# nagadomi/nunif

Hardware: NVIDIA H100
Metric: waifu2x_input_megapixels_per_sec (higher is better)
Workload: dtype f16

## Files before the change

nunif_b200/csrc/gemm_wgmma.cuh:

```cuda
#pragma once
#include "common.cuh"
#include <cuda.h>

namespace nb200 {

enum : int { ACT_NONE = 0, ACT_LRELU01 = 1, ACT_GELU = 2, ACT_RELU = 3 };
enum : int { OUT_NHWC = 0, OUT_PIXSHUF2 = 1, OUT_SPLIT = 2 };

struct GemmParams {
    int B, Ho, Wo, TH, TW, tiles_x, tiles_y;
    int N;
    int taps, cpt;
    int8_t tap_dx[16], tap_dy[16], tap_dyi[16];
    int n_tiles;
    const float* bias;
    int act;
    int out_mode, cout;
    int has_res, res_cy, res_cx;
    int res_before_act;
};

struct GemmMaps {
    CUtensorMap a, b;
    CUtensorMap o[4];
    CUtensorMap r[4];
};

__device__ __forceinline__ uint32_t smem_u32(const void* p) { return (uint32_t)__cvta_generic_to_shared(p); }

__device__ __forceinline__ void mbar_init(uint64_t* bar, uint32_t count) {
    asm volatile("mbarrier.init.shared::cta.b64 [%0], %1;" ::"r"(smem_u32(bar)), "r"(count));
}
__device__ __forceinline__ void mbar_expect_tx(uint64_t* bar, uint32_t bytes) {
    asm volatile("mbarrier.arrive.expect_tx.shared::cta.b64 _, [%0], %1;" ::"r"(smem_u32(bar)), "r"(bytes) : "memory");
}
__device__ __forceinline__ void mbar_arrive(uint64_t* bar) {
    asm volatile("mbarrier.arrive.shared::cta.b64 _, [%0];" ::"r"(smem_u32(bar)) : "memory");
}
static __device__ __noinline__ void mbar_timeout() {
    printf("nb200: mbarrier wait timed out (block %d,%d thread %d)\n", blockIdx.x, blockIdx.y, threadIdx.x);
    __trap();
}
__device__ __forceinline__ void mbar_wait(uint64_t* bar, uint32_t parity) {
    const uint32_t addr = smem_u32(bar);
    uint32_t done = 0;
#pragma unroll 1
    for (uint32_t it = 0; it < (1u << 18); ++it) {
        asm volatile(
            "{\n\t.reg .pred p;\n\t"
            "mbarrier.try_wait.parity.shared::cta.b64 p, [%1], %2, %3;\n\t"
            "selp.u32 %0, 1, 0, p;\n\t}"
            : "=r"(done) : "r"(addr), "r"(parity), "r"(20000u) : "memory");
        if (done) return;
    }
    mbar_timeout();
}
__device__ __forceinline__ void fence_barrier_init() {
    asm volatile("fence.mbarrier_init.release.cluster;" ::: "memory");
    asm volatile("fence.proxy.async.shared::cta;" ::: "memory");
}
__device__ __forceinline__ void tma_load_5d(const CUtensorMap* map, uint64_t* bar, void* dst, int c0, int c1, int c2, int c3, int c4) {
    asm volatile(
        "cp.async.bulk.tensor.5d.shared::cluster.global.tile.mbarrier::complete_tx::bytes [%0], [%1, {%3, %4, %5, %6, %7}], [%2];"
        ::"r"(smem_u32(dst)), "l"(map), "r"(smem_u32(bar)), "r"(c0), "r"(c1), "r"(c2), "r"(c3), "r"(c4) : "memory");
}
__device__ __forceinline__ void tma_load_2d(const CUtensorMap* map, uint64_t* bar, void* dst, int c0, int c1) {
    asm volatile(
        "cp.async.bulk.tensor.2d.shared::cluster.global.tile.mbarrier::complete_tx::bytes [%0], [%1, {%3, %4}], [%2];"
        ::"r"(smem_u32(dst)), "l"(map), "r"(smem_u32(bar)), "r"(c0), "r"(c1) : "memory");
}
__device__ __forceinline__ void tma_load_4d(const CUtensorMap* map, uint64_t* bar, void* dst, int c0, int c1, int c2, int c3) {
    asm volatile(
        "cp.async.bulk.tensor.4d.shared::cluster.global.tile.mbarrier::complete_tx::bytes [%0], [%1, {%3, %4, %5, %6}], [%2];"
        ::"r"(smem_u32(dst)), "l"(map), "r"(smem_u32(bar)), "r"(c0), "r"(c1), "r"(c2), "r"(c3) : "memory");
}
__device__ __forceinline__ void tma_store_4d(const CUtensorMap* map, const void* src, int c0, int c1, int c2, int c3) {
    asm volatile("cp.async.bulk.tensor.4d.global.shared::cta.tile.bulk_group [%0, {%2, %3, %4, %5}], [%1];"
                 ::"l"(map), "r"(smem_u32(src)), "r"(c0), "r"(c1), "r"(c2), "r"(c3) : "memory");
// ... 282 lines not shown
```

nunif_b200/csrc/model.cu:

```cuda
#include "common.cuh"
#include "gemm.h"
#include "gemm_wgmma.cuh"
#include "swin_kernels.h"
#include "cunet_kernels.h"
#include "legacy_kernels.h"
#include "depth_kernels.h"
#include "rowflow_kernels.h"
#include "depth_aa_kernels.h"
#include "mlbw_kernels.h"
#include "zoe_kernels.h"
#include "inpaint_kernels.h"
#include "window_mha.h"
#include "sod_kernels.h"
#include "../../include/nunif_b200.h"
#include <map>
#include <vector>
#include <string>
#include <cstring>
#include <cmath>
#include <memory>
#include <tuple>
#include <algorithm>

namespace nb200 {
// ... 260 lines not shown
        Arena size;
        plan(size);
        if (ensure_ws(size.off + 4096)) return 1;
        Arena a{ws};
        plan(a);
        return 0;
    }
};

namespace nb200 {

static void pack_swin_blocks(Packer& pk, std::vector<SwinBlockW>& out, const std::string& prefix, int C, int layers) {
    for (int i = 0; i < layers; ++i) {
        SwinBlockW b;
        const std::string p = prefix + ".block." + std::to_string(i);
        b.C = C;
        b.shift = (i % 2 == 0) ? 0 : 3;
        b.qkv = pack_linear(pk, p + ".attn.qkv", 3 * C, C);
        b.proj = pack_linear(pk, p + ".attn.proj", C, C);
        b.fc1 = pack_linear(pk, p + ".mlp.0", 2 * C, C);
        b.fc2 = pack_linear(pk, p + ".mlp.3", C, 2 * C);
        const float* t = pk.get(p + ".attn.relative_position_bias_table", 121 * 6);
        if (t) {
            std::vector<float> frag(BIAS_FRAG_FLOATS);
            for (int head = 0; head < 6; ++head)
                for (int mt = 0; mt < 3; ++mt)
                    for (int nt = 0; nt < 6; ++nt)
                        for (int lane = 0; lane < 32; ++lane)
                            for (int r = 0; r < 4; ++r) {
                                const int g = lane >> 2, t4 = lane & 3;
                                const int row = mt * 16 + g + 8 * (r >> 1), col = nt * 8 + 2 * t4 + (r & 1);
                                float v;
                                if (col >= 36) v = -1e30f;
                                else if (row >= 36) v = 0.f;
                                else {
                                    const int qy = row / 6, qx = row % 6, ky = col / 6, kx = col % 6;
                                    v = 1.4426950408889634f * t[((qy - ky + 5) * 11 + (qx - kx + 5)) * 6 + head];
                                }
                                frag[((((size_t)head * 3 + mt) * 6 + nt) * 32 + lane) * 4 + r] = v;
                            }
            b.table = pk.add_f32(frag);
        }
        pk.mark(p + ".attn.relative_position_index");
        out.push_back(b);
    }
}

static void pack_swin(Packer& pk, SwinW& w, int r) {
    const int C = 96;
    w.C = C;
    w.r = r;
    w.cs = (3 * r * r + 15) / 16 * 16;
    w.stem = pack_stem(pk, "unet.patch.0", C / 2, 64);
    w.conv2 = pack_conv(pk, "unet.patch.2", C, C / 2, 3, 3, 64);
    pack_swin_blocks(pk, w.s1, "unet.swin1", C, 2);
    w.down1 = pack_conv(pk, "unet.down1.conv", 2 * C, C, 2, 2);
    pack_swin_blocks(pk, w.s2, "unet.swin2", 2 * C, 2);
    w.down2 = pack_conv(pk, "unet.down2.conv", 2 * C, 2 * C, 2, 2);
    pack_swin_blocks(pk, w.s3, "unet.swin3", 2 * C, 6);
    w.up2 = pack_linear_pixshuf2(pk, "unet.up2.proj", 2 * C, 2 * C);
    pack_swin_blocks(pk, w.s4, "unet.swin4", 2 * C, 2);
    if (r == 4) {
        w.proj2 = pack_linear(pk, "unet.proj2", 2 * C, C);
        w.up1 = pack_linear_pixshuf2(pk, "unet.up1.proj", 2 * C, 2 * C);
// ... 473 lines not shown
```

nunif_b200/csrc/swin_attention_mma.cu:

```cuda
#include "common.cuh"
#include "gemm_wgmma.cuh"
#include "swin_kernels.h"
#include "tmap.h"
#include <map>
#include <mutex>

namespace nb200 {

extern int g_tune[16];

namespace {
constexpr int WS = 6, WTOK = 36, WPAD = 48, HEADS = 6;

__device__ __forceinline__ void mma16816(float (&c)[4], const uint32_t (&a)[4], uint32_t b0, uint32_t b1) {
    asm volatile(
        "mma.sync.aligned.m16n8k16.row.col.f32.f16.f16.f32 {%0,%1,%2,%3}, {%4,%5,%6,%7}, {%8,%9}, {%0,%1,%2,%3};"
        : "+f"(c[0]), "+f"(c[1]), "+f"(c[2]), "+f"(c[3])
        : "r"(a[0]), "r"(a[1]), "r"(a[2]), "r"(a[3]), "r"(b0), "r"(b1));
}
__device__ __forceinline__ void ldmatrix_x2_trans(uint32_t& r0, uint32_t& r1, const void* smem_row) {
    const uint32_t addr = (uint32_t)__cvta_generic_to_shared(smem_row);
    asm volatile("ldmatrix.sync.aligned.m8n8.x2.trans.shared.b16 {%0,%1}, [%2];" : "=r"(r0), "=r"(r1) : "r"(addr));
}
__device__ __forceinline__ uint32_t pack_half2(float a, float b) {
// ... 255 lines not shown
int window_attention(cudaStream_t st, const __half* qkv, const float* bias_frag_f, __half* out, int B, int H, int W, int C,
                     int shift, size_t plane) {
    const float4* bias_table = reinterpret_cast<const float4*>(bias_frag_f);
    NB_CHECK(H % WS == 0 && W % WS == 0, "feature map must be a multiple of the 6x6 window");
    NB_CHECK(C == 96 || C == 192, "window attention supports C=96 (d=16) and C=192 (d=32)");
    if (WS >= H) shift = 0;
    dim3 grid((H / WS) * (W / WS), B);
    ProfScope ps(st, PC_ATTN, (double)B * H * W * C * 4 * 2, (double)B * H * W * C * 3 * 2, (double)B * H * W * C * 2);
    if (C == 96) {
        const int want = g_tune[6] > 0 ? g_tune[6] : 72;
        if (set_attn_attrs((const void*)window_attention_mma_kernel<16>, attn_smem_bytes<16>(), want)) return 1;
        window_attention_mma_kernel<16><<<grid, 192, attn_smem_bytes<16>(), st>>>(qkv, bias_table, out, H, W, shift, plane);
    } else {
        const int want = g_tune[6] > 0 ? g_tune[6] : 86;
        if (set_attn_attrs((const void*)window_attention_mma_kernel<32>, attn_smem_bytes<32>(), want)) return 1;
        window_attention_mma_kernel<32><<<grid, 192, attn_smem_bytes<32>(), st>>>(qkv, bias_table, out, H, W, shift, plane);
    }
    NB_LAUNCHED();
    return 0;
}


constexpr int FA_ROWS = 128, FA_WIN = 3, FA_THREADS = GEMM_CONSUMER_THREADS + 32, FA_SLOT = 96 * 64, FA_STAGES = 4;
constexpr int FA_LD = 32 + 8;
constexpr int FA_CHUNK_BYTES = FA_WIN * 3 * WTOK * FA_LD * 2;

template <int C>
struct FaCfg {
    static constexpr int X_BYTES = FA_ROWS * C * 2;
    static constexpr int SMEM = X_BYTES + FA_STAGES * FA_SLOT + FA_CHUNK_BYTES + FA_WIN * (WTOK + WPAD) * 4 + 2 * FA_STAGES * 8 + 1024;
};

template <int C>
__global__ void __launch_bounds__(FA_THREADS, 2) swin_attn_fused_kernel(const __grid_constant__ CUtensorMap wmap,
                                                                        const __half* __restrict__ x, const float* __restrict__ bqkv,
                                                                        const float4* __restrict__ bias_frag, __half* __restrict__ out,
                                                                        int H, int W, int shift, int nwin) {
    using Cfg = FaCfg<C>;
    constexpr int D = C / HEADS, KB = C / 32, NCH = C / 32, HPC = 32 / D;
    extern __shared__ uint8_t smem_dyn[];
    uint8_t* smem = reinterpret_cast<uint8_t*>((reinterpret_cast<uintptr_t>(smem_dyn) + 1023) & ~(uintptr_t)1023);
    uint8_t* sx = smem;
    uint8_t* ring = smem + Cfg::X_BYTES;
    __half* sqkv = reinterpret_cast<__half*>(ring + FA_STAGES * FA_SLOT);
    int* stok = reinterpret_cast<int*>(reinterpret_cast<uint8_t*>(sqkv) + FA_CHUNK_BYTES);
    int* sreg = stok + FA_WIN * WTOK;
    uint64_t* full = reinterpret_cast<uint64_t*>(sreg + FA_WIN * WPAD);
    uint64_t* empty = full + FA_STAGES;
    const int tid = threadIdx.x, warp = tid >> 5;
    const int nww = W / WS, nwy = H / WS;
    if (tid < FA_WIN * WPAD) {
        const int w = tid / WPAD, t = tid % WPAD, gw = blockIdx.x * FA_WIN + w;
        int reg = -1;
        if (t < WTOK) {
            int tok = -1;
            if (gw < nwin) {
                const int b = gw / (nww * nwy), r = gw % (nww * nwy), wy = r / nww, wx = r % nww;
                const int ry = wy * WS + t / WS, rx = wx * WS + t % WS;
                const int y = (ry + shift) % H, xx = (rx + shift) % W;
                tok = (b * H + y) * W + xx;
                int hr = 0, wr = 0;
                if (shift > 0) {
                    hr = ry < H - WS ? 0 : (ry < H - shift ? 1 : 2);
                    wr = rx < W - WS ? 0 : (rx < W - shift ? 1 : 2);
                }
                reg = hr * 3 + wr;
            }
            stok[w * WTOK + t] = tok;
// ... 12 lines not shown
    if (tid == 0) NB_PDL_TRIGGER();

    if (warp == GEMM_CONSUMER_THREADS / 32) {
        if (elect_one()) {
            for (int i = 0; i < NCH * KB; ++i) {
                const int s = i % FA_STAGES, c = i / KB;
                mbar_wait(&empty[s], ((i / FA_STAGES) & 1) ^ 1);
                mbar_expect_tx(&full[s], FA_SLOT);
#pragma unroll
                for (int m = 0; m < 3; ++m)
                    tma_load_2d(&wmap, &full[s], ring + s * FA_SLOT + m * 32 * 64, (i % KB) * 32, m * C + 32 * c);
            }
        }
        return;
    }

    for (int i = tid; i < FA_ROWS * (C / 8); i += GEMM_CONSUMER_THREADS) {
        const int r = i / (C / 8), u = i % (C / 8);
        uint8_t* dst = sx + (u >> 2) * (FA_ROWS * 64) + stage_off<32>(r, u & 3);
        const int tok = r < FA_WIN * WTOK ? stok[r] : -1;
        if (tok >= 0) cp_async16(dst, x + (size_t)tok * C + u * 8);
        else *reinterpret_cast<uint4*>(dst) = make_uint4(0u, 0u, 0u, 0u);
    }
    asm volatile("cp.async.commit_group;" ::: "memory");
    asm volatile("cp.async.wait_group 0;" ::: "memory");
    fence_async_smem();
    consumer_bar_sync();

    const int wg = tid >> 7, t = tid & 127;
    const int row0 = wg * 64 + (t >> 5) * 16 + ((t & 31) >> 2);
    const int cq = 2 * (t & 3);
    const uint32_t a_base = smem_u32(sx) + wg * 64 * 64;
    const int lane = tid & 31, g = lane >> 2, t4 = lane & 3;
    const float scale = ((D == 16) ? 0.25f : 0.17677669529663687f) * 1.4426950408889634f;
#pragma unroll 1
    for (int c = 0; c < NCH; ++c) {
        float acc[48];
#pragma unroll
        for (int j = 0; j < 48; ++j) acc[j] = 0.f;
#pragma unroll 1
        for (int kb = 0; kb < KB; ++kb) {
            const int it = c * KB + kb, s = it % FA_STAGES;
            mbar_wait(&full[s], (it / FA_STAGES) & 1);
            const uint32_t a = a_base + kb * (FA_ROWS * 64), bb = smem_u32(ring + s * FA_SLOT);
            wgmma_fence();
            wgmma_f16<96>(acc, make_kmajor_desc<64>(a), make_kmajor_desc<64>(bb), 1u);
            wgmma_f16<96>(acc, make_kmajor_desc<64>(a + 32), make_kmajor_desc<64>(bb + 32), 1u);
            wgmma_commit();
            wgmma_wait<1>();
            if (kb > 0 && t == 0) mbar_arrive(&empty[(it - 1) % FA_STAGES]);
        }
        wgmma_wait<0>();
        if (t == 0) mbar_arrive(&empty[(c * KB + KB - 1) % FA_STAGES]);
        wgmma_fence_operands(acc);
        consumer_bar_sync();
#pragma unroll
        for (int j = 0; j < 12; ++j) {
            const int m = j >> 2, col = 8 * (j & 3) + cq;
            const float2 bq = __ldg(reinterpret_cast<const float2*>(bqkv + m * C + 32 * c + col));
#pragma unroll
            for (int i = 0; i < 2; ++i) {
                const int r = row0 + 8 * i;
                if (r < FA_WIN * WTOK) {
                    const int w = r / WTOK, tk = r - w * WTOK;
                    *reinterpret_cast<__half2*>(sqkv + ((w * 3 + m) * WTOK + tk) * FA_LD + col) =
                        __floats2half2_rn(acc[4 * j + 2 * i] + bq.x, acc[4 * j + 2 * i + 1] + bq.y);
                }
            }
        }
        consumer_bar_sync();

#pragma unroll 1
        for (int item = warp; item < 3 * FA_WIN * HPC; item += GEMM_CONSUMER_THREADS / 32) {
            const int mt = item / (FA_WIN * HPC), pr = item - mt * (FA_WIN * HPC), w = pr / HPC, hh = pr - w * HPC;
            const int gw = blockIdx.x * FA_WIN + w;
            if (gw >= nwin) continue;
            const int r = gw % (nww * nwy), wy = r / nww, wx = r % nww, head = c * HPC + hh;
            __half* sq = sqkv + w * 3 * WTOK * FA_LD;
            __half* sk = sq + WTOK * FA_LD;
            __half* sv = sk + WTOK * FA_LD;
            AttnCtx<D> cx;
            cx.sq = sq; cx.sreg = sreg + w * WPAD; cx.bf = bias_frag + (size_t)head * (3 * 6 * 32) + lane;
            cx.hc = hh * D; cx.g = g; cx.t4 = t4; cx.scale = scale;
            cx.boundary = shift > 0 && (wy == nwy - 1 || wx == nww - 1);
#pragma unroll
            for (int nt = 0; nt < NKT; ++nt) cx.kbase[nt] = sk + min(nt * 8 + g, WTOK - 1) * FA_LD + cx.hc + 2 * t4;
            cx.vbase[0] = sv + (lane & 15) * FA_LD + cx.hc;
            cx.vbase[1] = sv + (16 + (lane & 15)) * FA_LD + cx.hc;
            cx.vbase[2] = sv + min(32 + (lane & 7), WTOK - 1) * FA_LD + cx.hc;
            if (mt < 2) attn_mtile<D, FA_LD, false>(cx, mt);
            else attn_mtile<D, FA_LD, true>(cx, 2);
            __syncwarp();
            const int nrow = mt < 2 ? 16 : WTOK - 32;
            for (int e = lane; e < nrow * (D / 8); e += 32) {
                const int tk = 16 * mt + e / (D / 8), u = e % (D / 8);
                *reinterpret_cast<uint4*>(out + (size_t)stok[w * WTOK + tk] * C + head * D + u * 8) =
                    *reinterpret_cast<const uint4*>(sq + tk * FA_LD + cx.hc + u * 8);
            }
        }
    }
}

int swin_attn_fused(cudaStream_t st, const __half* x, const __half* wqkv, const float* bqkv, const float* bias_frag_f, __half* att,
                    int B, int H, int W, int C, int shift) {
    NB_CHECK(x && wqkv && bqkv && bias_frag_f && att, "null pointer");
    NB_CHECK(H % WS == 0 && W % WS == 0, "feature map must be a multiple of the 6x6 window");
    NB_CHECK(C == 96 || C == 192, "fused window attention supports C=96 (d=16) and C=192 (d=32)");
    if (WS >= H) shift = 0;
    const long long nwin = (long long)B * (H / WS) * (W / WS);
    NB_CHECK(nwin > 0 && nwin < (1LL << 31), "window count out of range");
    CUtensorMap wmap;
    const cuuint64_t dims[2] = {(cuuint64_t)C, (cuuint64_t)(3 * C)};
    const cuuint64_t strides[1] = {(cuuint64_t)C * 2};
    const cuuint32_t box[2] = {32, 32};
    if (encode(&wmap, wqkv, 2, dims, strides, box, 64)) return 1;
    const double T = (double)B * H * W;
    ProfScope ps(st, PC_FUSED_ATTN, T * 3.0 * C * C * 2 + T * C * 36 * 4, T * C * 2, T * C * 2);
    const unsigned grid = (unsigned)((nwin + FA_WIN - 1) / FA_WIN);
    const float4* bf = reinterpret_cast<const float4*>(bias_frag_f);
    if (C == 96) {
        if (ensure_dyn_smem((const void*)swin_attn_fused_kernel<96>, FaCfg<96>::SMEM)) return 1;
        swin_attn_fused_kernel<96><<<grid, FA_THREADS, FaCfg<96>::SMEM, st>>>(wmap, x, bqkv, bf, att, H, W, shift, (int)nwin);
    } else {
        if (ensure_dyn_smem((const void*)swin_attn_fused_kernel<192>, FaCfg<192>::SMEM)) return 1;
        swin_attn_fused_kernel<192><<<grid, FA_THREADS, FaCfg<192>::SMEM, st>>>(wmap, x, bqkv, bf, att, H, W, shift, (int)nwin);
    }
    NB_LAUNCHED();
    return 0;
}

}
```

nunif_b200/csrc/swin_block.cu:

```cuda
#include "gemm_wgmma.cuh"
#include "swin_kernels.h"
#include "tmap.h"

namespace nb200 {

constexpr int FM_ROWS = 128, FM_STAGES = 5, FM_THREADS = GEMM_CONSUMER_THREADS + 128;
constexpr int FM_PRODUCER_REGS = 40, FM_CONSUMER_REGS = 232;

template <int C>
struct FmCfg {
    static constexpr int KB = C / 32;
    static constexpr int TILE = FM_ROWS * C * 2;
    static constexpr int STAGE = 128 * C;
    static constexpr int SMEM = 2 * TILE + FM_STAGES * STAGE + (2 * FM_STAGES + KB + 1) * 8 + 1024;
};

struct FmMaps {
    CUtensorMap x, att, wp, w1, w2;
};

template <int K>
__device__ __forceinline__ float (&half96(float (&acc)[K], int h))[48] { return *reinterpret_cast<float(*)[48]>(&acc[48 * h]); }

__device__ __forceinline__ void fm_wait(uint64_t* bar, uint32_t parity) {
    const uint32_t addr = smem_u32(bar);
    uint32_t done = 0;
#pragma unroll 1
    for (uint32_t it = 0; it < (1u << 18) && !done; ++it)
        asm volatile(
            "{\n\t.reg .pred p;\n\t"
            "mbarrier.try_wait.parity.shared::cta.b64 p, [%1], %2, %3;\n\t"
            "selp.u32 %0, 1, 0, p;\n\t}"
            : "=r"(done) : "r"(addr), "r"(parity), "r"(20000u) : "memory");
    if (!done) __trap();
}

__device__ __forceinline__ void wgmma_wait_n(int n) {
    if (n == 0) wgmma_wait<0>();
    else wgmma_wait<1>();
}

template <int C, bool PROJ>
__global__ void __launch_bounds__(FM_THREADS, 1) swin_mlp_fused_kernel(const __grid_constant__ FmMaps maps, const float* __restrict__ bp,
                                                                     const float* __restrict__ b1, const float* __restrict__ b2) {
    using Cfg = FmCfg<C>;
    constexpr int KB = Cfg::KB, NP = (KB + 1) / 2, NH = 2 * C / 64, NHALF = C / 96;
    extern __shared__ uint8_t smem_dyn[];
    uint8_t* smem = reinterpret_cast<uint8_t*>((reinterpret_cast<uintptr_t>(smem_dyn) + 1023) & ~(uintptr_t)1023);
    uint8_t* sx = smem;
    uint8_t* satt = smem + Cfg::TILE;
    uint8_t* ring = smem + 2 * Cfg::TILE;
    uint64_t* full = reinterpret_cast<uint64_t*>(ring + FM_STAGES * Cfg::STAGE);
    uint64_t* empty = full + FM_STAGES;
    uint64_t* abar = empty + FM_STAGES;
    uint64_t* xbar = abar + KB;
    const int tid = threadIdx.x, warp = tid >> 5;
    const int row_base = blockIdx.x * FM_ROWS;
    if (tid == GEMM_CONSUMER_THREADS) {
// ... 13 lines not shown
        fence_barrier_init();
    }
    __syncthreads();

    if (warp >= GEMM_CONSUMER_THREADS / 32) {
        asm volatile("setmaxnreg.dec.sync.aligned.u32 %0;" ::"n"(FM_PRODUCER_REGS));
        if (warp == GEMM_CONSUMER_THREADS / 32 && elect_one()) {
            bool acts = false;
            auto load_acts = [&]() {
                asm volatile("griddepcontrol.wait;" ::: "memory");
                if (PROJ)
                    for (int kb = 0; kb < KB; ++kb) {
                        mbar_expect_tx(&abar[kb], FM_ROWS * 64);
                        tma_load_2d(&maps.att, &abar[kb], satt + kb * (FM_ROWS * 64), kb * 32, row_base);
                    }
                mbar_expect_tx(xbar, Cfg::TILE);
                for (int kb = 0; kb < KB; ++kb) tma_load_2d(&maps.x, xbar, sx + kb * (FM_ROWS * 64), kb * 32, row_base);
                acts = true;
            };
            int it = 0;
            auto push = [&](const CUtensorMap* m, int k0, int n0, int rows, int nbox) {
                if (it == FM_STAGES) load_acts();
                const int s = it % FM_STAGES;
                fm_wait(&empty[s], ((it / FM_STAGES) & 1) ^ 1);
                mbar_expect_tx(&full[s], nbox * rows * 64);
                for (int b = 0; b < nbox; ++b) tma_load_2d(m, &full[s], ring + s * Cfg::STAGE + b * rows * 64, k0 + 32 * b, n0);
                ++it;
            };
            if (PROJ)
                for (int j = 0; j < NP; ++j) push(&maps.wp, 64 * j, 0, C, min(2, KB - 2 * j));
            push(&maps.w1, 0, 0, 64, KB);
            for (int hc = 0; hc < NH; ++hc) {
                if (hc + 1 < NH) push(&maps.w1, 0, (hc + 1) * 64, 64, KB);
                push(&maps.w2, hc * 64, 0, C, 2);
            }
            if (!acts) load_acts();
        }
        return;
    }

    asm volatile("setmaxnreg.inc.sync.aligned.u32 %0;" ::"n"(FM_CONSUMER_REGS));
    const int wg = tid >> 7, t = tid & 127;
    const int row0 = wg * 64 + (t >> 5) * 16 + ((t & 31) >> 2);
    const int cq = 2 * (t & 3);
    const uint32_t x_base = smem_u32(sx) + wg * 64 * 64, att_base = smem_u32(satt) + wg * 64 * 64;
    int it = 0, pending = 0;
    auto take = [&]() -> uint32_t {
        const int s = it % FM_STAGES;
        fm_wait(&full[s], (it / FM_STAGES) & 1);
        return smem_u32(ring + s * Cfg::STAGE);
    };
    auto commit = [&]() {
        wgmma_commit();
        ++it;
        ++pending;
    };
    auto retire = [&](int n) {
        wgmma_wait_n(n);
#pragma unroll
        for (int k = 0; k < FM_STAGES; ++k)
            if (k < pending - n && t == 0) mbar_arrive(&empty[(it - pending + k) % FM_STAGES]);
        pending = min(pending, n);
    };

    if (PROJ) {
        float acc[C / 2];
#pragma unroll
        for (int j = 0; j < C / 2; ++j) acc[j] = 0.f;
        wgmma_fence_operands(acc);
#pragma unroll
        for (int j = 0; j < NP; ++j) {
            const uint32_t bb = take();
#pragma unroll
            for (int kb = 2 * j; kb < 2 * j + 2 && kb < KB; ++kb) fm_wait(&abar[kb], 0);
            wgmma_fence();
#pragma unroll
            for (int kb = 2 * j; kb < 2 * j + 2 && kb < KB; ++kb) {
                const uint32_t a = att_base + kb * (FM_ROWS * 64), b = bb + (kb - 2 * j) * (C * 64);
#pragma unroll
                for (int s = 0; s < 2; ++s)
#pragma unroll
                    for (int h = 0; h < NHALF; ++h)
                        wgmma_f16<96>(half96(acc, h), make_kmajor_desc<64>(a + 32 * s), make_kmajor_desc<64>(b + h * 96 * 64 + 32 * s), 1u);
            }
            commit();
            retire(1);
        }
        retire(0);
        wgmma_fence_operands(acc);
        fm_wait(xbar, 0);
#pragma unroll
        for (int j = 0; j < C / 8; ++j) {
            const int col = 8 * j + cq;
            const float2 bq = __ldg(reinterpret_cast<const float2*>(bp + col));
#pragma unroll
            for (int i = 0; i < 2; ++i) {
                __half2* p = reinterpret_cast<__half2*>(sx + sw64_off<FM_ROWS>(row0 + 8 * i, col));
                const float2 xv = __half22float2(*p);
                *p = __floats2half2_rn(xv.x + (acc[4 * j + 2 * i] + bq.x), xv.y + (acc[4 * j + 2 * i + 1] + bq.y));
            }
        }
        fence_async_smem();
        asm volatile("bar.sync %0, 128;" ::"r"(2 + wg) : "memory");
    } else {
        fm_wait(xbar, 0);
    }

    float oacc[C / 2];
#pragma unroll
    for (int j = 0; j < C / 2; ++j) oacc[j] = 0.f;
    wgmma_fence_operands(oacc);
    float hacc[2][32];
    uint32_t af[4][4];
    auto fc1 = [&](float (&h)[32]) {
#pragma unroll
        for (int j = 0; j < 32; ++j) h[j] = 0.f;
        wgmma_fence_operands(h);
        const uint32_t bb = take();
        wgmma_fence();
#pragma unroll
        for (int kb = 0; kb < KB; ++kb) {
            const uint32_t a = x_base + kb * (FM_ROWS * 64), b = bb + kb * (64 * 64);
            wgmma_f16<64>(h, make_kmajor_desc<64>(a), make_kmajor_desc<64>(b), 1u);
            wgmma_f16<64>(h, make_kmajor_desc<64>(a + 32), make_kmajor_desc<64>(b + 32), 1u);
        }
        commit();
    };
    fc1(hacc[0]);
// ... 78 lines not shown
    if (att && (map2d(&maps.att, att, C, T, FM_ROWS) || map2d(&maps.wp, wp, C, C, C))) return 1;
    if (map2d(&maps.w1, w1, C, 2 * C, 64) || map2d(&maps.w2, w2, 2 * C, C, C)) return 1;
    const double Td = (double)T;
    ProfScope ps(st, PC_FUSED_MLP, Td * C * C * 2 * ((att ? 1 : 0) + 4), Td * C * 2 * (att ? 2 : 1), Td * C * 2);
    const unsigned grid = (unsigned)((T + FM_ROWS - 1) / FM_ROWS);
    if (C == 96) return att ? launch_mlp<96, true>(st, grid, maps, bp, b1, b2) : launch_mlp<96, false>(st, grid, maps, bp, b1, b2);
    return att ? launch_mlp<192, true>(st, grid, maps, bp, b1, b2) : launch_mlp<192, false>(st, grid, maps, bp, b1, b2);
}

}

using namespace nb200;

extern "C" int nb200_swin_mlp_fused_f16(void* x, const void* att, long long T, int C, const void* wp, const float* bp,
                                        const void* w1, const float* b1, const void* w2, const float* b2, void* stream) {
    return swin_mlp_fused((cudaStream_t)stream, (__half*)x, (const __half*)att, T, C, (const __half*)wp, bp, (const __half*)w1, b1,
                          (const __half*)w2, b2);
}

extern "C" int nb200_swin_attn_fused_f16(const void* x, const void* wqkv, const float* bqkv, const float* bias_table, void* att,
                                         int B, int H, int W, int C, int shift, void* stream) {
    NB_CHECK(bias_table, "null pointer");
    cudaStream_t st = (cudaStream_t)stream;
    float* frag = nullptr;
    NB_CUDA(cudaMallocAsync((void**)&frag, BIAS_FRAG_FLOATS * sizeof(float), st));
    int rc = build_bias_frag(st, bias_table, frag);
    if (!rc) rc = swin_attn_fused(st, (const __half*)x, (const __half*)wqkv, bqkv, frag, (__half*)att, B, H, W, C, shift);
    cudaFreeAsync(frag, st);
    return rc;
}
```

nunif_b200/csrc/swin_kernels.h:

```cpp
#pragma once
#include "common.cuh"

namespace nb200 {
int stem_conv3x3(cudaStream_t st, const __half* x, const float* wt, const float* bias, __half* out, int n, int Hi, int Wi,
                 int cout_pad, int ldo);
constexpr int BIAS_FRAG_FLOATS = 6 * 3 * 6 * 32 * 4;
int build_bias_frag(cudaStream_t st, const float* table_121x6, float* frag);
int window_attention(cudaStream_t st, const __half* qkv, const float* bias_frag, __half* out, int B, int H, int W, int C,
                     int shift, size_t plane);
int swin_attn_fused(cudaStream_t st, const __half* x, const __half* wqkv, const float* bqkv, const float* bias_frag, __half* att,
                    int B, int H, int W, int C, int shift);
int swin_mlp_fused(cudaStream_t st, __half* x, const __half* att, long long T, int C, const __half* wp, const float* bp,
                   const __half* w1, const float* b1, const __half* w2, const float* b2);
int to_image(cudaStream_t st, const __half* y, void* z, int n, int Hs, int Ws, int cs, int r, int down);
}
```

profiles/ab_swin_attn.py:

```python
#!/usr/bin/env python
import argparse
import ctypes
import json
import os
import statistics
import subprocess
import sys
import tempfile

ROOT = os.path.dirname(os.path.dirname(os.path.abspath(__file__)))
sys.path.insert(0, ROOT)

SHAPES = [(240, 96), (120, 192), (60, 192), (240, 192)]
BATCH = 16
REPS = 7
WINDOW_MS = 60.0
FA_THREADS = 288
KERNEL = "_ZN5nb20022swin_attn_fused_kernelILi{C}EEEv14CUtensorMap_stPK6__halfPKfPK6float4PS2_iiii"


def load(path):
    from nunif_b200 import _lib
    lib = ctypes.CDLL(os.path.abspath(path))
    for name in ("nb200_last_error", "nb200_check_device", "nb200_swin_attn_fused_f16"):
        res, args = _lib.SIGNATURES[name]
        getattr(lib, name).restype, getattr(lib, name).argtypes = res, args
    return lib


def check(lib, rc):
    if rc != 0:
        raise RuntimeError(lib.nb200_last_error().decode("utf-8", "replace"))


def call(lib, t, shift):
    import torch
    x, wqkv, bqkv, table, att = t
    B, H, W, C = x.shape
    p = lambda v: ctypes.c_void_p(v.data_ptr())
    check(lib, lib.nb200_swin_attn_fused_f16(p(x), p(wqkv), p(bqkv), p(table), p(att), B, H, W, C, shift,
                                             ctypes.c_void_p(torch.cuda.current_stream().cuda_stream)))
# ... 22 lines not shown

def launch_smem(libs, dev):
    import torch
    from torch.profiler import ProfilerActivity, profile
    out = {}
    with tempfile.TemporaryDirectory() as d:
        for tag, lib in libs.items():
            for C in (96, 192):
                x, wqkv, bqkv, table = inputs(12, C, 0, dev)
                t = (x, wqkv, bqkv, table, torch.empty_like(x))
                with profile(activities=[ProfilerActivity.CUDA]) as prof:
                    call(lib, t, 0)
                    torch.cuda.synchronize()
                path = os.path.join(d, f"{tag}{C}.json")
                prof.export_chrome_trace(path)
                ev = [e for e in json.load(open(path))["traceEvents"]
                      if e.get("cat") == "kernel" and "swin_attn_fused_kernel" in e.get("name", "")]
                a = ev[0]["args"]
                out[(tag, C)] = {"smem": int(a["shared memory"]), "regs_trace": int(a["registers per thread"])}
    return out


def occupancy(so_path, C, smem):
    name = KERNEL.format(C=C)
    cuobjdump = os.path.join(os.environ.get("CUDA_HOME", "/usr/local/cuda"), "bin", "cuobjdump")
    with tempfile.TemporaryDirectory() as d:
        subprocess.run([cuobjdump, "-xelf", "all", os.path.abspath(so_path)], cwd=d, check=True, capture_output=True)
        image = next(b for b in (open(os.path.join(d, f), "rb").read() for f in sorted(os.listdir(d))) if name.encode() in b)
    cu = ctypes.CDLL("libcuda.so.1")

    def ck(rc):
        if rc != 0:
            raise RuntimeError(f"CUDA driver error {rc}")
    mod, fn = ctypes.c_void_p(), ctypes.c_void_p()
    ck(cu.cuModuleLoadData(ctypes.byref(mod), ctypes.c_char_p(image)))
    try:
        ck(cu.cuModuleGetFunction(ctypes.byref(fn), mod, name.encode()))
        ck(cu.cuFuncSetAttribute(fn, 8, ctypes.c_int(smem)))
        regs, n = ctypes.c_int(), ctypes.c_int()
        ck(cu.cuFuncGetAttribute(ctypes.byref(regs), 4, fn))
        ck(cu.cuOccupancyMaxActiveBlocksPerMultiprocessor(ctypes.byref(n), fn, FA_THREADS, ctypes.c_size_t(smem)))
    finally:
        cu.cuModuleUnload(mod)
    return regs.value, n.value


def device_info(index):
    q = subprocess.run(["nvidia-smi", "-i", str(index), "--query-gpu=name,power.limit,clocks.max.sm", "--format=csv,noheader"],
                       capture_output=True, text=True)
    return q.stdout.strip()

# ... 70 lines not shown
```

Before: 53.31.

## Run fused Swin window attention on warpgroup wgmma with register-resident Q

Replaces the per-warp mma.sync window attention, which staged Q/K/V in a padded shared buffer, with warpgroup wgmma. Q stays in registers as the A operand, and K/V are written to double-buffered swizzled shared tiles so one consumer_bar_sync is dropped. Softmax now runs directly on the S accumulators using a precomputed dense bias table instead of fragment-ordered bias. The kernel is also templated on the shift flag so the unshifted case skips the mask work. This adds register pressure from 80-wide accumulators and extra zero-fill and shared memory for the KV buffers.

```diff
diff --git a/nunif_b200/csrc/gemm_wgmma.cuh b/nunif_b200/csrc/gemm_wgmma.cuh
--- a/nunif_b200/csrc/gemm_wgmma.cuh
+++ b/nunif_b200/csrc/gemm_wgmma.cuh
@@ -37,23 +37,17 @@
 __device__ __forceinline__ void mbar_arrive(uint64_t* bar) {
     asm volatile("mbarrier.arrive.shared::cta.b64 _, [%0];" ::"r"(smem_u32(bar)) : "memory");
 }
-static __device__ __noinline__ void mbar_timeout() {
-    printf("nb200: mbarrier wait timed out (block %d,%d thread %d)\n", blockIdx.x, blockIdx.y, threadIdx.x);
-    __trap();
-}
 __device__ __forceinline__ void mbar_wait(uint64_t* bar, uint32_t parity) {
     const uint32_t addr = smem_u32(bar);
     uint32_t done = 0;
 #pragma unroll 1
-    for (uint32_t it = 0; it < (1u << 18); ++it) {
+    for (uint32_t it = 0; it < (1u << 18) && !done; ++it)
         asm volatile(
             "{\n\t.reg .pred p;\n\t"
             "mbarrier.try_wait.parity.shared::cta.b64 p, [%1], %2, %3;\n\t"
             "selp.u32 %0, 1, 0, p;\n\t}"
             : "=r"(done) : "r"(addr), "r"(parity), "r"(20000u) : "memory");
-        if (done) return;
-    }
-    mbar_timeout();
+    if (!done) __trap();
 }
 __device__ __forceinline__ void fence_barrier_init() {
     asm volatile("fence.mbarrier_init.release.cluster;" ::: "memory");
diff --git a/nunif_b200/csrc/model.cu b/nunif_b200/csrc/model.cu
--- a/nunif_b200/csrc/model.cu
+++ b/nunif_b200/csrc/model.cu
@@ -306,24 +306,9 @@
         b.fc2 = pack_linear(pk, p + ".mlp.3", C, 2 * C);
         const float* t = pk.get(p + ".attn.relative_position_bias_table", 121 * 6);
         if (t) {
-            std::vector<float> frag(BIAS_FRAG_FLOATS);
-            for (int head = 0; head < 6; ++head)
-                for (int mt = 0; mt < 3; ++mt)
-                    for (int nt = 0; nt < 6; ++nt)
-                        for (int lane = 0; lane < 32; ++lane)
-                            for (int r = 0; r < 4; ++r) {
-                                const int g = lane >> 2, t4 = lane & 3;
-                                const int row = mt * 16 + g + 8 * (r >> 1), col = nt * 8 + 2 * t4 + (r & 1);
-                                float v;
-                                if (col >= 36) v = -1e30f;
-                                else if (row >= 36) v = 0.f;
-                                else {
-                                    const int qy = row / 6, qx = row % 6, ky = col / 6, kx = col % 6;
-                                    v = 1.4426950408889634f * t[((qy - ky + 5) * 11 + (qx - kx + 5)) * 6 + head];
-                                }
-                                frag[((((size_t)head * 3 + mt) * 6 + nt) * 32 + lane) * 4 + r] = v;
-                            }
-            b.table = pk.add_f32(frag);
+            std::vector<float> bias(ATTN_BIAS_FLOATS);
+            for (int i = 0; i < ATTN_BIAS_FLOATS; ++i) bias[i] = attn_bias_value(t, i);
+            b.table = pk.add_f32(bias);
         }
         pk.mark(p + ".attn.relative_position_index");
         out.push_back(b);
diff --git a/nunif_b200/csrc/swin_attention_mma.cu b/nunif_b200/csrc/swin_attention_mma.cu
--- a/nunif_b200/csrc/swin_attention_mma.cu
+++ b/nunif_b200/csrc/swin_attention_mma.cu
@@ -301,19 +301,51 @@
 
 
 constexpr int FA_ROWS = 128, FA_WIN = 3, FA_THREADS = GEMM_CONSUMER_THREADS + 32, FA_SLOT = 96 * 64, FA_STAGES = 4;
-constexpr int FA_LD = 32 + 8;
-constexpr int FA_CHUNK_BYTES = FA_WIN * 3 * WTOK * FA_LD * 2;
+constexpr int FA_KROWS = 40;
+constexpr int FA_KV_BYTES = 128 * 64;
+
+namespace {
+__device__ __forceinline__ void wgmma_rs_n80(float (&d)[40], const uint32_t (&a)[4], uint64_t b, uint32_t acc) {
+    asm volatile("{\n\t.reg .pred p;\n\tsetp.ne.b32 p, %45, 0;\n\t"
+                 "wgmma.mma_async.sync.aligned.m64n80k16.f32.f16.f16 {%0, %1, %2, %3, %4, %5, %6, %7, %8, %9, %10, %11, %12, %13, %14, %15, %16, %17, %18, %19, %20, %21, %22, %23, %24, %25, %26, %27, %28, %29, %30, %31, %32, %33, %34, %35, %36, %37, %38, %39}, {%40, %41, %42, %43}, %44, p, 1, 1, 0;\n\t}"
+                 : "+f"(d[0]), "+f"(d[1]), "+f"(d[2]), "+f"(d[3]), "+f"(d[4]), "+f"(d[5]), "+f"(d[6]), "+f"(d[7]), "+f"(d[8]), "+f"(d[9]), "+f"(d[10]), "+f"(d[11]), "+f"(d[12]), "+f"(d[13]), "+f"(d[14]), "+f"(d[15]), "+f"(d[16]), "+f"(d[17]), "+f"(d[18]), "+f"(d[19]), "+f"(d[20]), "+f"(d[21]), "+f"(d[22]), "+f"(d[23]), "+f"(d[24]), "+f"(d[25]), "+f"(d[26]), "+f"(d[27]), "+f"(d[28]), "+f"(d[29]), "+f"(d[30]), "+f"(d[31]), "+f"(d[32]), "+f"(d[33]), "+f"(d[34]), "+f"(d[35]), "+f"(d[36]), "+f"(d[37]), "+f"(d[38]), "+f"(d[39])
+                 : "r"(a[0]), "r"(a[1]), "r"(a[2]), "r"(a[3]), "l"(b), "r"(acc));
+}
+__device__ __forceinline__ void st_shared_if(uint32_t addr, uint32_t v, bool p) {
+    asm volatile("{\n\t.reg .pred q;\n\tsetp.ne.b32 q, %2, 0;\n\t@q st.shared.b32 [%0], %1;\n\t}" ::"r"(addr), "r"(v), "r"((int)p) : "memory");
+}
+__device__ __forceinline__ void st_global_if(void* ptr, uint32_t v, bool p) {
+    asm volatile("{\n\t.reg .pred q;\n\tsetp.ne.b32 q, %2, 0;\n\t@q st.global.b32 [%0], %1;\n\t}" ::"l"(ptr), "r"(v), "r"((int)p) : "memory");
+}
+__device__ __forceinline__ float sel_f32(bool p, float a, float b) {
+    float r;
+    asm("{\n\t.reg .pred q;\n\tsetp.ne.b32 q, %3, 0;\n\tselp.f32 %0, %1, %2, q;\n\t}" : "=f"(r) : "f"(a), "f"(b), "r"((int)p));
+    return r;
+}
+__device__ __forceinline__ uint32_t sel_b32(bool p, uint32_t a, uint32_t b) {
+    uint32_t r;
+    asm("{\n\t.reg .pred q;\n\tsetp.ne.b32 q, %3, 0;\n\tselp.b32 %0, %1, %2, q;\n\t}" : "=r"(r) : "r"(a), "r"(b), "r"((int)p));
+    return r;
+}
+__device__ __forceinline__ uint32_t h2_bits(__half2 h) { return *reinterpret_cast<const uint32_t*>(&h); }
+__device__ __forceinline__ void wgmma_rs_n32_tb(float (&d)[16], const uint32_t (&a)[4], uint64_t b, uint32_t acc) {
+    asm volatile("{\n\t.reg .pred p;\n\tsetp.ne.b32 p, %21, 0;\n\t"
+                 "wgmma.mma_async.sync.aligned.m64n32k16.f32.f16.f16 {%0, %1, %2, %3, %4, %5, %6, %7, %8, %9, %10, %11, %12, %13, %14, %15}, {%16, %17, %18, %19}, %20, p, 1, 1, 1;\n\t}"
+                 : "+f"(d[0]), "+f"(d[1]), "+f"(d[2]), "+f"(d[3]), "+f"(d[4]), "+f"(d[5]), "+f"(d[6]), "+f"(d[7]), "+f"(d[8]), "+f"(d[9]), "+f"(d[10]), "+f"(d[11]), "+f"(d[12]), "+f"(d[13]), "+f"(d[14]), "+f"(d[15])
+                 : "r"(a[0]), "r"(a[1]), "r"(a[2]), "r"(a[3]), "l"(b), "r"(acc));
+}
+}
 
 template <int C>
 struct FaCfg {
     static constexpr int X_BYTES = FA_ROWS * C * 2;
-    static constexpr int SMEM = X_BYTES + FA_STAGES * FA_SLOT + FA_CHUNK_BYTES + FA_WIN * (WTOK + WPAD) * 4 + 2 * FA_STAGES * 8 + 1024;
+    static constexpr int SMEM = X_BYTES + FA_STAGES * FA_SLOT + 4 * FA_KV_BYTES + FA_WIN * (WTOK + WPAD) * 4 + 2 * FA_STAGES * 8 + 1024;
 };
 
-template <int C>
+template <int C, bool SHIFTED>
 __global__ void __launch_bounds__(FA_THREADS, 2) swin_attn_fused_kernel(const __grid_constant__ CUtensorMap wmap,
                                                                         const __half* __restrict__ x, const float* __restrict__ bqkv,
-                                                                        const float4* __restrict__ bias_frag, __half* __restrict__ out,
+                                                                        const float* __restrict__ attn_bias, __half* __restrict__ out,
                                                                         int H, int W, int shift, int nwin) {
     using Cfg = FaCfg<C>;
     constexpr int D = C / HEADS, KB = C / 32, NCH = C / 32, HPC = 32 / D;
@@ -321,8 +353,8 @@
     uint8_t* smem = reinterpret_cast<uint8_t*>((reinterpret_cast<uintptr_t>(smem_dyn) + 1023) & ~(uintptr_t)1023);
     uint8_t* sx = smem;
     uint8_t* ring = smem + Cfg::X_BYTES;
-    __half* sqkv = reinterpret_cast<__half*>(ring + FA_STAGES * FA_SLOT);
-    int* stok = reinterpret_cast<int*>(reinterpret_cast<uint8_t*>(sqkv) + FA_CHUNK_BYTES);
+    uint8_t* skv = ring + FA_STAGES * FA_SLOT;
+    int* stok = reinterpret_cast<int*>(skv + 4 * FA_KV_BYTES);
     int* sreg = stok + FA_WIN * WTOK;
     uint64_t* full = reinterpret_cast<uint64_t*>(sreg + FA_WIN * WPAD);
     uint64_t* empty = full + FA_STAGES;
@@ -381,6 +413,8 @@
         if (tok >= 0) cp_async16(dst, x + (size_t)tok * C + u * 8);
         else *reinterpret_cast<uint4*>(dst) = make_uint4(0u, 0u, 0u, 0u);
     }
+    for (int i = tid; i < 4 * FA_KV_BYTES / 16; i += GEMM_CONSUMER_THREADS)
+        reinterpret_cast<uint4*>(skv)[i] = make_uint4(0u, 0u, 0u, 0u);
     asm volatile("cp.async.commit_group;" ::: "memory");
     asm volatile("cp.async.wait_group 0;" ::: "memory");
     fence_async_smem();
@@ -390,8 +424,15 @@
     const int row0 = wg * 64 + (t >> 5) * 16 + ((t & 31) >> 2);
     const int cq = 2 * (t & 3);
     const uint32_t a_base = smem_u32(sx) + wg * 64 * 64;
-    const int lane = tid & 31, g = lane >> 2, t4 = lane & 3;
+    const uint32_t kv_base = smem_u32(skv) + wg * FA_KROWS * 64;
     const float scale = ((D == 16) ? 0.25f : 0.17677669529663687f) * 1.4426950408889634f;
+    int tq[2], hf[2];
+#pragma unroll
+    for (int i = 0; i < 2; ++i) {
+        const int r = row0 + 8 * i, wq = min(r / WTOK, FA_WIN - 1);
+        tq[i] = min(r - wq * WTOK, WTOK - 1);
+        hf[i] = wq - wg;
+    }
 #pragma unroll 1
     for (int c = 0; c < NCH; ++c) {
         float acc[48];
@@ -412,57 +453,138 @@
         wgmma_wait<0>();
         if (t == 0) mbar_arrive(&empty[(c * KB + KB - 1) % FA_STAGES]);
         wgmma_fence_operands(acc);
-        consumer_bar_sync();
+        const uint32_t kvb = (c & 1) * 2 * FA_KV_BYTES, k_base = kv_base + kvb, v_base = k_base + FA_KV_BYTES;
+        uint32_t qa[2][4];
 #pragma unroll
         for (int j = 0; j < 12; ++j) {
             const int m = j >> 2, col = 8 * (j & 3) + cq;
             const float2 bq = __ldg(reinterpret_cast<const float2*>(bqkv + m * C + 32 * c + col));
 #pragma unroll
             for (int i = 0; i < 2; ++i) {
-                const int r = row0 + 8 * i;
-                if (r < FA_WIN * WTOK) {
-                    const int w = r / WTOK, tk = r - w * WTOK;
-                    *reinterpret_cast<__half2*>(sqkv + ((w * 3 + m) * WTOK + tk) * FA_LD + col) =
-                        __floats2half2_rn(acc[4 * j + 2 * i] + bq.x, acc[4 * j + 2 * i + 1] + bq.y);
+                const uint32_t h = h2_bits(__floats2half2_rn(acc[4 * j + 2 * i] + bq.x, acc[4 * j + 2 * i + 1] + bq.y));
+                if (m == 0) {
+                    qa[(j & 3) >> 1][2 * (j & 1) + i] = h;
+                } else {
+                    const int r = row0 + 8 * i, w = min(r / WTOK, FA_WIN - 1), kr = w * FA_KROWS + r - w * WTOK;
+                    st_shared_if(smem_u32(skv) + kvb + (m - 1) * FA_KV_BYTES + stage_off<32>(kr, col >> 3) + (col & 7) * 2, h, r < FA_WIN * WTOK);
                 }
             }
         }
+        fence_async_smem();
         consumer_bar_sync();
 
 #pragma unroll 1
-        for (int item = warp; item < 3 * FA_WIN * HPC; item += GEMM_CONSUMER_THREADS / 32) {
-            const int mt = item / (FA_WIN * HPC), pr = item - mt * (FA_WIN * HPC), w = pr / HPC, hh = pr - w * HPC;
-            const int gw = blockIdx.x * FA_WIN + w;
-            if (gw >= nwin) continue;
-            const int r = gw % (nww * nwy), wy = r / nww, wx = r % nww, head = c * HPC + hh;
-            __half* sq = sqkv + w * 3 * WTOK * FA_LD;
-            __half* sk = sq + WTOK * FA_LD;
-            __half* sv = sk + WTOK * FA_LD;
-            AttnCtx<D> cx;
-            cx.sq = sq; cx.sreg = sreg + w * WPAD; cx.bf = bias_frag + (size_t)head * (3 * 6 * 32) + lane;
-            cx.hc = hh * D; cx.g = g; cx.t4 = t4; cx.scale = scale;
-            cx.boundary = shift > 0 && (wy == nwy - 1 || wx == nww - 1);
-#pragma unroll
-            for (int nt = 0; nt < NKT; ++nt) cx.kbase[nt] = sk + min(nt * 8 + g, WTOK - 1) * FA_LD + cx.hc + 2 * t4;
-            cx.vbase[0] = sv + (lane & 15) * FA_LD + cx.hc;
-            cx.vbase[1] = sv + (16 + (lane & 15)) * FA_LD + cx.hc;
-            cx.vbase[2] = sv + min(32 + (lane & 7), WTOK - 1) * FA_LD + cx.hc;
-            if (mt < 2) attn_mtile<D, FA_LD, false>(cx, mt);
-            else attn_mtile<D, FA_LD, true>(cx, 2);
-            __syncwarp();
-            const int nrow = mt < 2 ? 16 : WTOK - 32;
-            for (int e = lane; e < nrow * (D / 8); e += 32) {
-                const int tk = 16 * mt + e / (D / 8), u = e % (D / 8);
-                *reinterpret_cast<uint4*>(out + (size_t)stok[w * WTOK + tk] * C + head * D + u * 8) =
-                    *reinterpret_cast<const uint4*>(sq + tk * FA_LD + cx.hc + u * 8);
+        for (int hh = 0; hh < HPC; ++hh) {
+            const int head = c * HPC + hh;
+            uint32_t qh[4];
+#pragma unroll
+            for (int q = 0; q < 4; ++q) qh[q] = sel_b32(hh == 0, qa[0][q], qa[1][q]);
+            float s[40];
+            wgmma_fence();
+#pragma unroll
+            for (int kk = 0; kk < D / 16; ++kk)
+                wgmma_rs_n80(s, D == 32 ? qa[kk] : qh, make_kmajor_desc<64>(k_base + 32 * (D == 32 ? kk : hh)), kk > 0 ? 1u : 0u);
+            wgmma_commit();
+            wgmma_wait<0>();
+            wgmma_fence_operands(s);
+            uint32_t ph[2][5];
+            float rsum[2];
+#pragma unroll
+            for (int i = 0; i < 2; ++i) {
+                const float* brow = attn_bias + ((size_t)head * WTOK + tq[i]) * FA_KROWS + cq;
+                float v[5][2];
+#pragma unroll
+                for (int jj = 0; jj < 5; ++jj) {
+                    const float2 bv = __ldg(reinterpret_cast<const float2*>(brow + 8 * jj));
+                    v[jj][0] = fmaf(sel_f32(hf[i], s[4 * (jj + 5) + 2 * i], s[4 * jj + 2 * i]), scale, bv.x);
+                    v[jj][1] = fmaf(sel_f32(hf[i], s[4 * (jj + 5) + 2 * i + 1], s[4 * jj + 2 * i + 1]), scale, bv.y);
+                }
+                if (SHIFTED) {
+                    const int* kreg = sreg + (hf[i] + wg) * WPAD;
+                    const int rq = kreg[tq[i]];
+#pragma unroll
+                    for (int jj = 0; jj < 5; ++jj)
+#pragma unroll
+                        for (int e = 0; e < 2; ++e)
+                            v[jj][e] += sel_f32(kreg[8 * jj + cq + e] != rq, -100.0f * 1.4426950408889634f, 0.f);
+                }
+                float mx = -1e30f;
+#pragma unroll
+                for (int jj = 0; jj < 5; ++jj) mx = fmaxf(mx, fmaxf(v[jj][0], v[jj][1]));
+                mx = fmaxf(mx, __shfl_xor_sync(0xffffffffu, mx, 1));
+                mx = fmaxf(mx, __shfl_xor_sync(0xffffffffu, mx, 2));
+                float sum = 0.f;
+#pragma unroll
+                for (int jj = 0; jj < 5; ++jj) {
+                    float p0, p1;
+                    asm("ex2.approx.ftz.f32 %0, %1;" : "=f"(p0) : "f"(v[jj][0] - mx));
+                    asm("ex2.approx.ftz.f32 %0, %1;" : "=f"(p1) : "f"(v[jj][1] - mx));
+                    const __half2 hp = __floats2half2_rn(p0, p1);
+                    const float2 pr = __half22float2(hp);
+                    sum += pr.x + pr.y;
+                    ph[i][jj] = *reinterpret_cast<const uint32_t*>(&hp);
+                }
+                sum += __shfl_xor_sync(0xffffffffu, sum, 1);
+                sum += __shfl_xor_sync(0xffffffffu, sum, 2);
+                rsum[i] = __fdividef(1.f, sum);
             }
-        }
-    }
-}
-
-int swin_attn_fused(cudaStream_t st, const __half* x, const __half* wqkv, const float* bqkv, const float* bias_frag_f, __half* att,
+            uint32_t pa[2][3][4];
+#pragma unroll
+            for (int h = 0; h < 2; ++h)
+#pragma unroll
+                for (int kk = 0; kk < 3; ++kk)
+#pragma unroll
+                    for (int q = 0; q < 4; ++q) {
+                        const int j = 2 * kk + (q >> 1), i = q & 1;
+                        pa[h][kk][q] = j < 5 ? sel_b32(hf[i] == h, ph[i][j], 0u) : 0u;
+                    }
+            float o[16];
+            wgmma_fence();
+#pragma unroll
+            for (int h = 0; h < 2; ++h)
+#pragma unroll
+                for (int kk = 0; kk < 3; ++kk)
+                    wgmma_rs_n32_tb(o, pa[h][kk], make_kmajor_desc<64>(v_base + (h * FA_KROWS + kk * 16) * 64), h + kk > 0 ? 1u : 0u);
+            wgmma_commit();
+            wgmma_wait<0>();
+            wgmma_fence_operands(o);
+#pragma unroll
+            for (int jj = 0; jj < (D == 32 ? 4 : 2); ++jj)
+#pragma unroll
+                for (int i = 0; i < 2; ++i) {
+                    const int j = D == 32 ? jj : 2 * hh + jj, r = row0 + 8 * i, tok = stok[min(r, FA_WIN * WTOK - 1)];
+                    const float o0 = D == 32 ? o[4 * jj + 2 * i] : sel_f32(hh == 0, o[4 * jj + 2 * i], o[4 * (jj + 2) + 2 * i]);
+                    const float o1 = D == 32 ? o[4 * jj + 2 * i + 1] : sel_f32(hh == 0, o[4 * jj + 2 * i + 1], o[4 * (jj + 2) + 2 * i + 1]);
+                    st_global_if(out + (size_t)max(tok, 0) * C + 32 * c + 8 * j + cq, h2_bits(__floats2half2_rn(o0 * rsum[i], o1 * rsum[i])),
+                                 r < FA_WIN * WTOK && tok >= 0);
+                }
+        }
+    }
+}
+
+__global__ void build_attn_bias_kernel(const float* __restrict__ table, float* __restrict__ bias) {
+    const int i = blockIdx.x * blockDim.x + threadIdx.x;
+    if (i < ATTN_BIAS_FLOATS) bias[i] = attn_bias_value(table, i);
+}
+
+int build_attn_bias(cudaStream_t st, const float* table, float* bias) {
+    build_attn_bias_kernel<<<(ATTN_BIAS_FLOATS + 255) / 256, 256, 0, st>>>(table, bias);
+    NB_LAUNCHED();
+    return 0;
+}
+
+template <int C, bool SHIFTED>
+static int launch_attn(cudaStream_t st, unsigned grid, const CUtensorMap& wmap, const __half* x, const float* bqkv, const float* attn_bias,
+                       __half* att, int H, int W, int shift, int nwin) {
+    if (ensure_dyn_smem((const void*)swin_attn_fused_kernel<C, SHIFTED>, FaCfg<C>::SMEM)) return 1;
+    swin_attn_fused_kernel<C, SHIFTED><<<grid, FA_THREADS, FaCfg<C>::SMEM, st>>>(wmap, x, bqkv, attn_bias, att, H, W, shift, nwin);
+    NB_LAUNCHED();
+    return 0;
+}
+
+int swin_attn_fused(cudaStream_t st, const __half* x, const __half* wqkv, const float* bqkv, const float* attn_bias, __half* att,
                     int B, int H, int W, int C, int shift) {
-    NB_CHECK(x && wqkv && bqkv && bias_frag_f && att, "null pointer");
+    NB_CHECK(x && wqkv && bqkv && attn_bias && att, "null pointer");
     NB_CHECK(H % WS == 0 && W % WS == 0, "feature map must be a multiple of the 6x6 window");
     NB_CHECK(C == 96 || C == 192, "fused window attention supports C=96 (d=16) and C=192 (d=32)");
     if (WS >= H) shift = 0;
@@ -476,16 +598,10 @@
     const double T = (double)B * H * W;
     ProfScope ps(st, PC_FUSED_ATTN, T * 3.0 * C * C * 2 + T * C * 36 * 4, T * C * 2, T * C * 2);
     const unsigned grid = (unsigned)((nwin + FA_WIN - 1) / FA_WIN);
-    const float4* bf = reinterpret_cast<const float4*>(bias_frag_f);
-    if (C == 96) {
-        if (ensure_dyn_smem((const void*)swin_attn_fused_kernel<96>, FaCfg<96>::SMEM)) return 1;
-        swin_attn_fused_kernel<96><<<grid, FA_THREADS, FaCfg<96>::SMEM, st>>>(wmap, x, bqkv, bf, att, H, W, shift, (int)nwin);
-    } else {
-        if (ensure_dyn_smem((const void*)swin_attn_fused_kernel<192>, FaCfg<192>::SMEM)) return 1;
-        swin_attn_fused_kernel<192><<<grid, FA_THREADS, FaCfg<192>::SMEM, st>>>(wmap, x, bqkv, bf, att, H, W, shift, (int)nwin);
-    }
-    NB_LAUNCHED();
-    return 0;
-}
-
-}
+    if (C == 96) return shift > 0 ? launch_attn<96, true>(st, grid, wmap, x, bqkv, attn_bias, att, H, W, shift, (int)nwin)
+                                  : launch_attn<96, false>(st, grid, wmap, x, bqkv, attn_bias, att, H, W, shift, (int)nwin);
+    return shift > 0 ? launch_attn<192, true>(st, grid, wmap, x, bqkv, attn_bias, att, H, W, shift, (int)nwin)
+                     : launch_attn<192, false>(st, grid, wmap, x, bqkv, attn_bias, att, H, W, shift, (int)nwin);
+}
+
+}
diff --git a/nunif_b200/csrc/swin_block.cu b/nunif_b200/csrc/swin_block.cu
--- a/nunif_b200/csrc/swin_block.cu
+++ b/nunif_b200/csrc/swin_block.cu
@@ -21,19 +21,6 @@
 
 template <int K>
 __device__ __forceinline__ float (&half96(float (&acc)[K], int h))[48] { return *reinterpret_cast<float(*)[48]>(&acc[48 * h]); }
-
-__device__ __forceinline__ void fm_wait(uint64_t* bar, uint32_t parity) {
-    const uint32_t addr = smem_u32(bar);
-    uint32_t done = 0;
-#pragma unroll 1
-    for (uint32_t it = 0; it < (1u << 18) && !done; ++it)
-        asm volatile(
-            "{\n\t.reg .pred p;\n\t"
-            "mbarrier.try_wait.parity.shared::cta.b64 p, [%1], %2, %3;\n\t"
-            "selp.u32 %0, 1, 0, p;\n\t}"
-            : "=r"(done) : "r"(addr), "r"(parity), "r"(20000u) : "memory");
-    if (!done) __trap();
-}
 
 __device__ __forceinline__ void wgmma_wait_n(int n) {
     if (n == 0) wgmma_wait<0>();
@@ -93,7 +80,7 @@
             auto push = [&](const CUtensorMap* m, int k0, int n0, int rows, int nbox) {
                 if (it == FM_STAGES) load_acts();
                 const int s = it % FM_STAGES;
-                fm_wait(&empty[s], ((it / FM_STAGES) & 1) ^ 1);
+                mbar_wait(&empty[s], ((it / FM_STAGES) & 1) ^ 1);
                 mbar_expect_tx(&full[s], nbox * rows * 64);
                 for (int b = 0; b < nbox; ++b) tma_load_2d(m, &full[s], ring + s * Cfg::STAGE + b * rows * 64, k0 + 32 * b, n0);
                 ++it;
@@ -118,7 +105,7 @@
     int it = 0, pending = 0;
     auto take = [&]() -> uint32_t {
         const int s = it % FM_STAGES;
-        fm_wait(&full[s], (it / FM_STAGES) & 1);
+        mbar_wait(&full[s], (it / FM_STAGES) & 1);
         return smem_u32(ring + s * Cfg::STAGE);
     };
     auto commit = [&]() {
@@ -143,7 +130,7 @@
         for (int j = 0; j < NP; ++j) {
             const uint32_t bb = take();
 #pragma unroll
-            for (int kb = 2 * j; kb < 2 * j + 2 && kb < KB; ++kb) fm_wait(&abar[kb], 0);
+            for (int kb = 2 * j; kb < 2 * j + 2 && kb < KB; ++kb) mbar_wait(&abar[kb], 0);
             wgmma_fence();
 #pragma unroll
             for (int kb = 2 * j; kb < 2 * j + 2 && kb < KB; ++kb) {
@@ -159,7 +146,7 @@
         }
         retire(0);
         wgmma_fence_operands(acc);
-        fm_wait(xbar, 0);
+        mbar_wait(xbar, 0);
 #pragma unroll
         for (int j = 0; j < C / 8; ++j) {
             const int col = 8 * j + cq;
@@ -174,7 +161,7 @@
         fence_async_smem();
         asm volatile("bar.sync %0, 128;" ::"r"(2 + wg) : "memory");
     } else {
-        fm_wait(xbar, 0);
+        mbar_wait(xbar, 0);
     }
 
     float oacc[C / 2];
@@ -299,10 +286,10 @@
                                          int B, int H, int W, int C, int shift, void* stream) {
     NB_CHECK(bias_table, "null pointer");
     cudaStream_t st = (cudaStream_t)stream;
-    float* frag = nullptr;
-    NB_CUDA(cudaMallocAsync((void**)&frag, BIAS_FRAG_FLOATS * sizeof(float), st));
-    int rc = build_bias_frag(st, bias_table, frag);
-    if (!rc) rc = swin_attn_fused(st, (const __half*)x, (const __half*)wqkv, bqkv, frag, (__half*)att, B, H, W, C, shift);
-    cudaFreeAsync(frag, st);
+    float* bias = nullptr;
+    NB_CUDA(cudaMallocAsync((void**)&bias, ATTN_BIAS_FLOATS * sizeof(float), st));
+    int rc = build_attn_bias(st, bias_table, bias);
+    if (!rc) rc = swin_attn_fused(st, (const __half*)x, (const __half*)wqkv, bqkv, bias, (__half*)att, B, H, W, C, shift);
+    cudaFreeAsync(bias, st);
     return rc;
 }
diff --git a/nunif_b200/csrc/swin_kernels.h b/nunif_b200/csrc/swin_kernels.h
--- a/nunif_b200/csrc/swin_kernels.h
+++ b/nunif_b200/csrc/swin_kernels.h
@@ -8,7 +8,16 @@
 int build_bias_frag(cudaStream_t st, const float* table_121x6, float* frag);
 int window_attention(cudaStream_t st, const __half* qkv, const float* bias_frag, __half* out, int B, int H, int W, int C,
                      int shift, size_t plane);
-int swin_attn_fused(cudaStream_t st, const __half* x, const __half* wqkv, const float* bqkv, const float* bias_frag, __half* att,
+
+constexpr int ATTN_BIAS_FLOATS = 6 * 36 * 40;
+__host__ __device__ inline float attn_bias_value(const float* table_121x6, int i) {
+    const int head = i / (36 * 40), q = (i / 40) % 36, k = i % 40;
+    if (k >= 36) return -1e30f;
+    const int qy = q / 6, qx = q % 6, ky = k / 6, kx = k % 6;
+    return 1.4426950408889634f * table_121x6[((qy - ky + 5) * 11 + (qx - kx + 5)) * 6 + head];
+}
+int build_attn_bias(cudaStream_t st, const float* table_121x6, float* attn_bias);
+int swin_attn_fused(cudaStream_t st, const __half* x, const __half* wqkv, const float* bqkv, const float* attn_bias, __half* att,
                     int B, int H, int W, int C, int shift);
 int swin_mlp_fused(cudaStream_t st, __half* x, const __half* att, long long T, int C, const __half* wp, const float* bp,
                    const __half* w1, const float* b1, const __half* w2, const float* b2);
diff --git a/profiles/ab_swin_attn.py b/profiles/ab_swin_attn.py
--- a/profiles/ab_swin_attn.py
+++ b/profiles/ab_swin_attn.py
@@ -3,6 +3,7 @@
 import ctypes
 import json
 import os
+import re
 import statistics
 import subprocess
 import sys
@@ -16,7 +17,7 @@
 REPS = 7
 WINDOW_MS = 60.0
 FA_THREADS = 288
-KERNEL = "_ZN5nb20022swin_attn_fused_kernelILi{C}EEEv14CUtensorMap_stPK6__halfPKfPK6float4PS2_iiii"
+KERNEL_RE = rb"_ZN5nb20022swin_attn_fused_kernelILi{C}E[A-Za-z0-9_]*?EEv14CUtensorMap_st[A-Za-z0-9_]+"
 
 
 def load(path):
@@ -85,11 +86,12 @@
 
 
 def occupancy(so_path, C, smem):
-    name = KERNEL.format(C=C)
+    name = KERNEL_RE.replace(b"{C}", str(C).encode())
     cuobjdump = os.path.join(os.environ.get("CUDA_HOME", "/usr/local/cuda"), "bin", "cuobjdump")
     with tempfile.TemporaryDirectory() as d:
         subprocess.run([cuobjdump, "-xelf", "all", os.path.abspath(so_path)], cwd=d, check=True, capture_output=True)
-        image = next(b for b in (open(os.path.join(d, f), "rb").read() for f in sorted(os.listdir(d))) if name.encode() in b)
+        image = next(b for b in (open(os.path.join(d, f), "rb").read() for f in sorted(os.listdir(d))) if re.search(name, b))
+        name = re.search(name, image).group(0).decode()
     cu = ctypes.CDLL("libcuda.so.1")
 
     def ck(rc):
```

Result: faster. 54.04, median of 6 (+1.4%).
